# yifita/pytorch_points

Measured on AMD Instinct MI355X. Metric: chamfer_fwd_bwd_point_pairs_per_s, higher is better.
Workload: dtype f32

## Files before the change

### pytorch_points_amd/csrc/grid_common.h

```cpp
#pragma once
#include "pp_common.h"

#ifndef PP_PHASE
#define PP_PHASE(n)
#endif

namespace pp {

constexpr int kGridMax = 32;
constexpr float kGridMinExtent = 0x1p-44f;
constexpr int kGridCells = kGridMax * kGridMax * kGridMax;
constexpr int kBuildThreads = 1024;

constexpr int kBuildSlabs = 4;

constexpr int kLayerWords = 40;
constexpr int kLayerPending = 36;
constexpr int kLayerCursor = 37;
constexpr int kLayerRouted = 38;
constexpr int kChunk = 256;
constexpr int kChunkMax = 256;
__host__ __device__ inline int zkey(float z) {
#if defined(__HIP_DEVICE_COMPILE__)
  const int o = __float_as_int(z);
#else
  int o;
  __builtin_memcpy(&o, &z, 4);
#endif
  return o ^ ((o >> 31) & 0x7fffffff);
}
__device__ __forceinline__ float zkey_inv(int k) { return __int_as_float(k ^ ((k >> 31) & 0x7fffffff)); }

struct GridSet {
  float minx, miny, minz, h, invh;
  int gx, gy, gz;
  int useless;
  int pad[3];
  int crowd[kBuildSlabs];
};
static_assert(sizeof(GridSet) == 64, "");

__device__ __forceinline__ bool grid_useless(const GridSet& g) {
  return g.useless != 0 || g.crowd[0] == 1 || g.crowd[1] == 1 || g.crowd[2] == 1 || g.crowd[3] == 1;
}
__device__ __forceinline__ bool grid_refined(const GridSet& g) {
  return g.crowd[0] == 2 || g.crowd[1] == 2 || g.crowd[2] == 2 || g.crowd[3] == 2;
}

constexpr int kCrowd = 128;
constexpr int kSubMaxAxis = 26;
constexpr int kSubMaxCells = 16384;
constexpr int kSubWaveCells = 1536;
constexpr int kBuildSlabCrowdMax = 1024;
struct SubGrid {
  float minx, miny, minz, h, invh;
  int gx, gy, gz;
};
static_assert(sizeof(SubGrid) == 32, "");
__host__ __device__ inline size_t sub_desc_slots(size_t npoints) { return npoints / kCrowd + 2; }

__device__ __forceinline__ int cell_coord(float p, float mn, float invh, int g) {
  const float f = (p - mn) * invh;
  const int c = (int)f;
  int r;
  asm("v_med3_i32 %0, %1, 0, %2" : "=v"(r) : "v"(c), "v"(g - 1));
  return r;
}

__device__ __forceinline__ int cell_linear(int cx, int cy, int cz, int gx, int gy) {
  int r;
  asm("v_mad_u32_u24 %0, %1, %2, %3\n\tv_mad_u32_u24 %0, %0, %4, %5"
      : "=&v"(r)
      : "v"(cz), "v"(gy), "v"(cy), "v"(gx), "v"(cx));
  return r;
}

__host__ __device__ inline int grid_build_counter_words(int nslab) {
  const int per = (kGridCells + nslab - 1) / nslab + 1;
  return (per + per / 32 + 1 + 3) & ~3;
}
__host__ __device__ inline size_t grid_build_lds_bytes(int nslab) {
  return ((size_t)grid_build_counter_words(nslab) + (size_t)kBuildThreads * 16) * sizeof(unsigned);
}

__device__ __forceinline__ int morton3(int x, int y, int z) {
  auto spread = [](unsigned v) {
    v = (v | (v << 8)) & 0x0000f00fu;
    v = (v | (v << 4)) & 0x000c30c3u;
    v = (v | (v << 2)) & 0x00249249u;
    return v;
  };
  return (int)(spread((unsigned)x) | (spread((unsigned)y) << 1) | (spread((unsigned)z) << 2));
}

__device__ __attribute__((noinline)) void grid_refine_cells(f4* __restrict__ sorted, f4* __restrict__ sorted2,
                                                            float* __restrict__ sorted_payload,
                                                            float* __restrict__ payload2,
                                                            unsigned* __restrict__ sub_start,
                                                            SubGrid* __restrict__ sub_desc, unsigned* s_cnt,
                                                            unsigned* s_part, float* s_box,
                                                            const unsigned (*s_clist)[2], unsigned ncrowd) {
  const int t = threadIdx.x;
  {
    {
      const int lane = t & 63, wave = t >> 6;
      constexpr unsigned kWaveMaxPoints = 2048;
      auto sub_geometry = [&](const float (&bmn)[6], unsigned n, int max_cells) {
        SubGrid sg;
        sg.minx = -bmn[0]; sg.miny = -bmn[1]; sg.minz = -bmn[2];
        const float sex = bmn[3] - sg.minx, sey = bmn[4] - sg.miny, sez = bmn[5] - sg.minz;
        const float semax = fmaxf(sex, fmaxf(sey, sez));
        int g2 = (int)cbrtf((float)n);
        g2 = g2 < 2 ? 2 : (g2 > kSubMaxAxis - 1 ? kSubMaxAxis - 1 : g2);
        sg.h = semax / (float)g2;
        if (!(sg.h > 0.0f) || !__builtin_isfinite(sg.h) || semax < kGridMinExtent) sg.h = 1.0f;
        sg.invh = 1.0f / sg.h;
        auto cells2 = [&](float e) {
          const int c = (int)(e * sg.invh) + 1;
          return c < 1 ? 1 : (c > kSubMaxAxis ? kSubMaxAxis : c);
        };
        sg.gx = cells2(sex); sg.gy = cells2(sey); sg.gz = cells2(sez);
        while ((long long)sg.gx * sg.gy * sg.gz > min((long long)max_cells, 2LL * n - 1)) {
          if (sg.gx >= sg.gy && sg.gx >= sg.gz) --sg.gx; else if (sg.gy >= sg.gz) --sg.gy; else --sg.gz;
        }
        return sg;
      };
      auto trim_box = [&](float (&bmn)[6], const float (&sm)[6], unsigned n) {
        const float inv_n = 1.0f / (float)n;
        float lo[3] = {-bmn[0], -bmn[1], -bmn[2]}, hi[3] = {bmn[3], bmn[4], bmn[5]};
        const float ext0 = fmaxf(hi[0] - lo[0], fmaxf(hi[1] - lo[1], hi[2] - lo[2]));
        float tl[3], th[3];
#pragma unroll
        for (int a = 0; a < 3; ++a) {
          const float c = 0.5f * (lo[a] + hi[a]);
          const float m = sm[a] * inv_n;
          const float var = fmaxf(sm[3 + a] * inv_n - m * m, 0.0f);
          const float sd = sqrtf(var);
          tl[a] = fmaxf(lo[a], c + m - 3.5f * sd);
          th[a] = fminf(hi[a], c + m + 3.5f * sd);
        }
        const float ext1 = fmaxf(th[0] - tl[0], fmaxf(th[1] - tl[1], th[2] - tl[2]));
        if (ext1 > 0.0f && ext1 < 0.75f * ext0) {
#pragma unroll
          for (int a = 0; a < 3; ++a) {
            bmn[a] = -tl[a];
            bmn[3 + a] = th[a];
          }
        }
      };
      auto cell2 = [](const SubGrid& sg, const f4& p) {
        return cell_linear(cell_coord(p.x, sg.minx, sg.invh, sg.gx), cell_coord(p.y, sg.miny, sg.invh, sg.gy),
                           cell_coord(p.z, sg.minz, sg.invh, sg.gz), sg.gx, sg.gy);
      };
      auto wave_sync = []() {
        __builtin_amdgcn_fence(__ATOMIC_ACQ_REL, "workgroup");
        __builtin_amdgcn_wave_barrier();
      };
      {
        unsigned* s_sub = s_cnt + (size_t)wave * kSubWaveCells;
        for (unsigned ci = wave; ci < ncrowd; ci += kBuildThreads / 64) {
          const unsigned start = s_clist[ci][0], n = s_clist[ci][1];
          if (n > kWaveMaxPoints) continue;
          auto for_points = [&](const f4* __restrict__ src, auto&& fn) {
            for (unsigned k0 = 0; k0 < n; k0 += 512u) {
              f4 q8[8];
#pragma unroll
              for (int u = 0; u < 8; ++u) q8[u] = src[start + min(k0 + 64u * (unsigned)u + (unsigned)lane, n - 1u)];
#pragma unroll
              for (int u = 0; u < 8; ++u) {
                const unsigned k = k0 + 64u * (unsigned)u + (unsigned)lane;
                if (k < n) fn(q8[u], k);
              }
            }
          };
          float bmn[6] = {-__builtin_inff(), -__builtin_inff(), -__builtin_inff(), -__builtin_inff(), -__builtin_inff(),
                          -__builtin_inff()};
          for_points(sorted, [&](const f4& q, unsigned) {
            bmn[0] = fmaxf(bmn[0], -q.x); bmn[1] = fmaxf(bmn[1], -q.y); bmn[2] = fmaxf(bmn[2], -q.z);
            bmn[3] = fmaxf(bmn[3], q.x); bmn[4] = fmaxf(bmn[4], q.y); bmn[5] = fmaxf(bmn[5], q.z);
          });
          wave_reduce6_dpp<false, 6>(bmn);
#pragma unroll
          for (int e = 0; e < 6; ++e) bmn[e] = __int_as_float(__builtin_amdgcn_readlane(__float_as_int(bmn[e]), 63));
          {
            const float c0 = 0.5f * (bmn[3] - bmn[0]), c1 = 0.5f * (bmn[4] - bmn[1]), c2 = 0.5f * (bmn[5] - bmn[2]);
            float sm[6] = {0.0f, 0.0f, 0.0f, 0.0f, 0.0f, 0.0f};
            for_points(sorted, [&](const f4& q, unsigned) {
              const float dx = q.x - c0, dy = q.y - c1, dz = q.z - c2;
              sm[0] += dx; sm[1] += dy; sm[2] += dz;
              sm[3] = __builtin_fmaf(dx, dx, sm[3]); sm[4] = __builtin_fmaf(dy, dy, sm[4]); sm[5] = __builtin_fmaf(dz, dz, sm[5]);
            });
            wave_reduce6_dpp<true, 6>(sm);
#pragma unroll
            for (int e = 0; e < 6; ++e) sm[e] = __int_as_float(__builtin_amdgcn_readlane(__float_as_int(sm[e]), 63));
            trim_box(bmn, sm, n);
          }
          const SubGrid sg = sub_geometry(bmn, n, kSubWaveCells);
          const int total2 = sg.gx * sg.gy * sg.gz;
          for (int c = lane; c < total2; c += 64) s_sub[c] = 0u;
          wave_sync();
          for_points(sorted, [&](const f4& q, unsigned) { atomicAdd(&s_sub[cell2(sg, q)], 1u); });
          wave_sync();
          {
            const int per2 = (total2 + 63) / 64;
            const int d0 = min(total2, lane * per2), d1 = min(total2, d0 + per2);
            unsigned sum2 = 0;
            for (int c = d0; c < d1; ++c) sum2 += s_sub[c];
            unsigned incl2 = sum2;
#pragma unroll
            for (int off = 1; off < 64; off <<= 1) {
              const unsigned o = __shfl_up(incl2, off);
              if (lane >= off) incl2 += o;
            }
            unsigned run2 = start + incl2 - sum2;
            unsigned* __restrict__ tbl = sub_start + 2 * (size_t)start;
            for (int c = d0; c < d1; ++c) {
              const unsigned v = s_sub[c];
              s_sub[c] = run2;
              tbl[c] = run2;
              run2 += v;
            }
            if (lane == 0) tbl[total2] = start + n;
          }
          wave_sync();
          for_points(sorted, [&](const f4& q, unsigned k) {
            const unsigned pos = atomicAdd(&s_sub[cell2(sg, q)], 1u);
// ... 696 lines not shown
constexpr int kFastLdsCnt = 0;
constexpr int kFastLdsList = kFastLdsCnt + kFastCells + 64;
constexpr int kFastLdsTz = kFastLdsList + (kFastCap + 64) * 4;
constexpr int kFastLdsBox = kFastLdsTz + 2 * kChunkMax;
constexpr int kFastLdsPart = kFastLdsBox + (kBuildThreads / 64) * 16;
constexpr int kFastLdsClist = kFastLdsPart + 64;
constexpr int kFastLdsPlan = kFastLdsClist + 2 * kFastCrowdMax;
constexpr int kFastLdsWords = kFastLdsPlan + 16;
static_assert(sizeof(BuildPlan) <= 16 * 4, "");
__host__ __device__ inline size_t grid_build_fast_lds_bytes() { return (size_t)kFastLdsWords * 4; }

template <bool REFINE = true>
__device__ __forceinline__ int grid_build_set_fast(const float* __restrict__ ref, int nr, GridSet* gs,
                                                   unsigned* __restrict__ cell_start, f4* __restrict__ sorted,
                                                   unsigned* lds, int slab, unsigned* __restrict__ sub_start,
                                                   SubGrid* __restrict__ sub_desc, f4* __restrict__ sorted2,
                                                   int* __restrict__ tile_z, int tz_chunks,
                                                   unsigned* __restrict__ layers) {
  constexpr int KP = 16, nslab = kBuildSlabs;
  const int nchunkq = (nr + kChunk - 1) / kChunk;
  if (nr > kFastMaxPoints || nr < 4 * kBuildThreads || (nr & 3) != 0 || cell_start == nullptr) return 1;
  if (REFINE && (tile_z == nullptr || layers == nullptr || sub_start == nullptr || sub_desc == nullptr ||
                 nchunkq > tz_chunks || tz_chunks > kChunkMax))
    return 1;
  const int t = threadIdx.x, lane = t & 63, wave = __builtin_amdgcn_readfirstlane(t >> 6);
  unsigned* s_cnt = lds + kFastLdsCnt;
  f4* s_list = reinterpret_cast<f4*>(lds + kFastLdsList);
  unsigned* s_occ = lds + kFastLdsList;
  int* s_tz = reinterpret_cast<int*>(lds + kFastLdsTz);
  float* s_box = reinterpret_cast<float*>(lds + kFastLdsBox);
  unsigned* s_part = lds + kFastLdsPart;
  unsigned(*s_clist)[2] = reinterpret_cast<unsigned(*)[2]>(lds + kFastLdsClist);
  unsigned& s_below = s_part[33];
  unsigned& s_ncrowd = s_part[34];

  PP_PHASE(0);
  float px[KP], py[KP], pz[KP];
  bool live[KP / 4];
#pragma unroll
  for (int gq = 0; gq < KP / 4; ++gq) {
    const int p0 = gq * (4 * kBuildThreads) + 4 * t;
    live[gq] = p0 < nr;
    const f4* __restrict__ src = reinterpret_cast<const f4*>(ref + 3 * (size_t)(live[gq] ? p0 : 0));
    const f4 a = src[0], b = src[1], c = src[2];
    px[4 * gq] = a.x; py[4 * gq] = a.y; pz[4 * gq] = a.z;
    px[4 * gq + 1] = a.w; py[4 * gq + 1] = b.x; pz[4 * gq + 1] = b.y;
    px[4 * gq + 2] = b.z; py[4 * gq + 2] = b.w; pz[4 * gq + 2] = c.x;
    px[4 * gq + 3] = c.y; py[4 * gq + 3] = c.z; pz[4 * gq + 3] = c.w;
  }
  auto kidx = [&](int i) { return (i >> 2) * (4 * kBuildThreads) + 4 * t + (i & 3); };
  if (REFINE && t < 2 * kChunkMax) s_tz[t] = (t & 1) ? zkey(-__builtin_inff()) : zkey(__builtin_inff());
  if (t == 0) {
    s_ncrowd = 0u;
    s_below = 0u;
  }
  s_occ[t] = 0u;
  for (int c = 4 * t; c < kFastCells; c += 4 * kBuildThreads) *reinterpret_cast<uint4*>(&s_cnt[c]) = make_uint4(0u, 0u, 0u, 0u);
  float mnx = __builtin_inff(), mny = mnx, mnz = mnx, mxx = -mnx, mxy = -mnx, mxz = -mnx;
  float sm[6] = {0.0f, 0.0f, 0.0f, 0.0f, 0.0f, 0.0f};
#pragma unroll
  for (int i = 0; i < KP; ++i) {
    const float x = px[i], y = py[i], z = pz[i];
    mnx = fminf(mnx, x); mny = fminf(mny, y); mnz = fminf(mnz, z);
    mxx = fmaxf(mxx, x); mxy = fmaxf(mxy, y); mxz = fmaxf(mxz, z);
    if (live[i >> 2]) {
      sm[0] += x; sm[1] += y; sm[2] += z;
      sm[3] = __builtin_fmaf(x, x, sm[3]); sm[4] = __builtin_fmaf(y, y, sm[4]); sm[5] = __builtin_fmaf(z, z, sm[5]);
    }
  }
  PP_PHASE(1);
  bool any_bad;
  {
    float v[6] = {-mnx, -mny, -mnz, mxx, mxy, mxz};
    wave_reduce6_dpp<false, 6>(v);
    wave_reduce6_dpp<true, 6>(sm);
    if (lane == 63) {
#pragma unroll
      for (int e = 0; e < 6; ++e) s_box[wave * 16 + e] = v[e];
#pragma unroll
      for (int e = 0; e < 6; ++e) s_box[wave * 16 + 8 + e] = sm[e];
    }
    __syncthreads();
#pragma unroll
    for (int e = 0; e < 6; ++e) v[e] = s_box[(t & 15) * 16 + e];
#pragma unroll
    for (int e = 0; e < 6; ++e) sm[e] = s_box[(t & 15) * 16 + 8 + e];
    wave_reduce6_dpp<false, 4>(v);
    wave_reduce6_dpp<true, 4>(sm);
#pragma unroll
    for (int e = 0; e < 6; ++e) v[e] = __int_as_float(__builtin_amdgcn_readlane(__float_as_int(v[e]), 15));
#pragma unroll
    for (int e = 0; e < 6; ++e) sm[e] = __int_as_float(__builtin_amdgcn_readlane(__float_as_int(sm[e]), 15));
    mnx = -v[0]; mny = -v[1]; mnz = -v[2]; mxx = v[3]; mxy = v[4]; mxz = v[5];
    any_bad = !__builtin_isfinite(sm[3] + sm[4] + sm[5]);
  }
  float n_live = (float)nr;
  if (!REFINE && any_bad) {
    plain_finite_plan(ref, nr, s_box);
    auto uni = [&](int e) { return __int_as_float(__builtin_amdgcn_readfirstlane(__float_as_int(s_box[e]))); };
    mnx = -uni(0); mny = -uni(1); mnz = -uni(2); mxx = uni(3); mxy = uni(4); mxz = uni(5);
#pragma unroll
    for (int e = 0; e < 6; ++e) sm[e] = uni(8 + e);
    n_live = uni(14);
    any_bad = !(n_live > 0.0f) || !__builtin_isfinite(sm[3] + sm[4] + sm[5]);
    __syncthreads();
  }
  PP_PHASE(2);
  bool trimmed = false;
  float zmean = 0.0f, zsig = 0.0f;
  if (!any_bad) {
    const float inv_n = 1.0f / n_live;
    const float mean[3] = {sm[0] * inv_n, sm[1] * inv_n, sm[2] * inv_n};
    float sig[3];
#pragma unroll
    for (int a = 0; a < 3; ++a) sig[a] = sqrtf(fmaxf(sm[3 + a] * inv_n - mean[a] * mean[a], 0.0f));
    zmean = mean[2];
    zsig = sig[2];
    const bool stretched = mxx - mean[0] > 6.0f * sig[0] || mean[0] - mnx > 6.0f * sig[0] ||
                           mxy - mean[1] > 6.0f * sig[1] || mean[1] - mny > 6.0f * sig[1] ||
                           mxz - mean[2] > 6.0f * sig[2] || mean[2] - mnz > 6.0f * sig[2];
    if (stretched) {
      float w[6] = {-__builtin_inff(), -__builtin_inff(), -__builtin_inff(), -__builtin_inff(), -__builtin_inff(),
                    -__builtin_inff()};
#pragma unroll
      for (int i = 0; i < KP; ++i) {
        const float x = px[i], y = py[i], z = pz[i];
        const bool in = fabsf(x - mean[0]) <= 4.0f * sig[0] && fabsf(y - mean[1]) <= 4.0f * sig[1] &&
                        fabsf(z - mean[2]) <= 4.0f * sig[2];
        if (in) {
          w[0] = fmaxf(w[0], -x); w[1] = fmaxf(w[1], -y); w[2] = fmaxf(w[2], -z);
          w[3] = fmaxf(w[3], x); w[4] = fmaxf(w[4], y); w[5] = fmaxf(w[5], z);
        }
      }
#pragma unroll
      for (int e = 0; e < 6; ++e) w[e] = wave_reduce_dpp<false>(w[e]);
      __syncthreads();
      if (lane == 0)
#pragma unroll
        for (int e = 0; e < 6; ++e) s_box[wave * 16 + e] = w[e];
      __syncthreads();
#pragma unroll
      for (int e = 0; e < 6; ++e) w[e] = wave_reduce_dpp<false>(s_box[(t & 15) * 16 + e]);
      if (w[3] > -w[0] || w[4] > -w[1] || w[5] > -w[2]) {
        mnx = -w[0]; mny = -w[1]; mnz = -w[2]; mxx = w[3]; mxy = w[4]; mxz = w[5];
        trimmed = true;
      }
    }
  }
  PP_PHASE(3);
  const float ex = mxx - mnx, ey = mxy - mny, ez = mxz - mnz;
  const float emax = fmaxf(ex, fmaxf(ey, ez));
  if (any_bad || !(emax > 0.0f) || !__builtin_isfinite(emax) || emax < kGridMinExtent) return 1;
  int g0 = 1;
  while (g0 < kGridMax && g0 * g0 * g0 < 2 * nr) ++g0;
  float h, invh;
  int gx, gy, gz;
  auto set_resolution = [&](int g) {
    h = emax / (float)g;
    if (!(h > 0.0f) || !__builtin_isfinite(h)) h = 1.0f;
    invh = 1.0f / h;
    auto cells = [&](float e) {
      int c = (int)(e * invh) + 1;
      return c < 1 ? 1 : (c > kGridMax ? kGridMax : c);
    };
    gx = cells(ex); gy = cells(ey); gz = cells(ez);
  };
  set_resolution(g0);
  unsigned key[KP];
  int gxy = 0, lo = 0, ncs = 0;
  auto count_pass = [&](bool mark) {
    float ox = mnx, oy = mny, oz = mnz;
    asm volatile("" : "+s"(ox), "+s"(oy), "+s"(oz));
    unsigned nbelow = 0;
#pragma unroll
    for (int gq = 0; gq < KP / 4; ++gq) {
      int c4[4];
#pragma unroll
      for (int u = 0; u < 4; ++u) {
        const int i = 4 * gq + u;
        c4[u] = cell_linear(cell_coord(px[i], ox, invh, gx), cell_coord(py[i], oy, invh, gy),
                            cell_coord(pz[i], oz, invh, gz), gx, gy);
      }
      const bool alive = live[gq];
      const bool same4 = alive & (c4[0] == c4[1]) & (c4[1] == c4[2]) & (c4[2] == c4[3]);
      const int lead = __builtin_amdgcn_readfirstlane(c4[0]);
      if (__all(same4 && c4[0] == lead)) {
        const unsigned slot = (unsigned)(lead - lo);
        if (mark && lane == 0) atomicOr(&s_occ[lead >> 5], 1u << (lead & 31));
        if (lead < lo) nbelow += 256u;
        unsigned b0 = 0u;
        const bool mine = slot < (unsigned)ncs;
        if (mine && lane == 0) b0 = atomicAdd(&s_cnt[slot], 256u);
        b0 = (unsigned)__builtin_amdgcn_readfirstlane((int)b0) + 4u * (unsigned)lane;
#pragma unroll
        for (int u = 0; u < 4; ++u) key[4 * gq + u] = mine ? (slot | ((b0 + (unsigned)u) << 16)) : ~0u;
      } else {
#pragma unroll
        for (int u = 0; u < 4; ++u) {
          const int c = c4[u];
          if (mark) atomicOr(&s_occ[c >> 5], 1u << (c & 31));
          const unsigned slot = (unsigned)(c - lo);
          const bool mine = alive & (slot < (unsigned)ncs);
          nbelow += (unsigned)__builtin_popcountll(__ballot(alive & (c < lo)));
          const unsigned r = atomicAdd(&s_cnt[mine ? slot : (unsigned)(kFastCells + lane)], 1u);
          key[4 * gq + u] = mine ? (slot | (r << 16)) : ~0u;
        }
      }
    }
    if (lane == 0 && nbelow) atomicAdd(&s_below, nbelow);
  };
  unsigned running = 0, own = 0;
#if PP_BUILD_BALANCE
  const bool balance_z = fabsf(zsig - 0.2887f * ez) > 0.03f * ez || fabsf(zmean - (mnz + 0.5f * ez)) > 0.06f * ez;
#endif
  {
    constexpr int kRounds = 4;
    for (int round = 0;; ++round) {
      if (gz < kFastMinLayers) return 1;
      gxy = gx * gy;
      int zl = gz * slab / nslab, zh = gz * (slab + 1) / nslab;
#if PP_BUILD_BALANCE
      if (balance_z) {
        unsigned* s_hist = reinterpret_cast<unsigned*>(s_box);
        if (t < 32) s_hist[t] = 0u;
        __syncthreads();
#pragma unroll
        for (int gq = 0; gq < KP / 4; ++gq)
          if (live[gq]) atomicAdd(&s_hist[cell_coord(pz[4 * gq], mnz, invh, gz)], 1u);
        __syncthreads();
        const unsigned cum = wave_scan_u32_dpp(lane < gz ? s_hist[lane] : 0u);
        const unsigned tot = (unsigned)__builtin_amdgcn_readlane((int)cum, 63);
        int zb[nslab + 1];
        zb[0] = 0;
        zb[nslab] = gz;
#pragma unroll
        for (int k = 1; k < nslab; ++k)
          zb[k] = min(max((int)__builtin_popcountll(__ballot(lane < gz && (unsigned)nslab * cum <= (unsigned)k * tot)), zb[k - 1] + 1),
                      gz - (nslab - k));
        bool fits = true;
#pragma unroll
        for (int k = 0; k < nslab; ++k) fits = fits && (zb[k + 1] - zb[k]) * gxy <= kFastCells;
        if (fits) {
#pragma unroll
          for (int k = 0; k < nslab; ++k)
            if (k == slab) {
              zl = zb[k];
              zh = zb[k + 1];
            }
        }
      }
#endif
      lo = zl * gxy;
      ncs = (zh - zl) * gxy;
      const int nwords = (gxy * gz + 31) / 32;
      if (round > 0) {
        if (t < nwords) s_occ[t] = 0u;
        for (int c = 4 * t; c < ((ncs + 7) & ~7); c += 4 * kBuildThreads)
          *reinterpret_cast<uint4*>(&s_cnt[c]) = make_uint4(0u, 0u, 0u, 0u);
        if (t == 0) s_below = 0u;
        __syncthreads();
      }
      PP_PHASE(4);
      count_pass(round < kRounds);
      __syncthreads();
      PP_PHASE(5);
      unsigned v8[8];
      const int c0 = 8 * t;
      if (c0 < ncs) {
        const uint4 a = *reinterpret_cast<const uint4*>(&s_cnt[c0]);
        const uint4 b = *reinterpret_cast<const uint4*>(&s_cnt[c0 + 4]);
        v8[0] = a.x; v8[1] = a.y; v8[2] = a.z; v8[3] = a.w; v8[4] = b.x; v8[5] = b.y; v8[6] = b.z; v8[7] = b.w;
      } else {
#pragma unroll
        for (int u = 0; u < 8; ++u) v8[u] = 0u;
      }
      unsigned sum = 0;
#pragma unroll
      for (int u = 0; u < 8; ++u) sum += v8[u];
      const unsigned incl = wave_scan_u32_dpp(sum);
      const unsigned occ = wave_scan_u32_dpp(round < kRounds && t < nwords ? (unsigned)__builtin_popcount(s_occ[t]) : 0u);
      if (lane == 63) {
        s_part[wave] = incl;
        s_part[16 + wave] = occ;
      }
      __syncthreads();
      const unsigned tot16 = wave_scan_u32_dpp(s_part[lane & 15]);
      const unsigned occ16 = wave_scan_u32_dpp(s_part[16 + (lane & 15)]);
      const unsigned nocc = (unsigned)__builtin_amdgcn_readlane((int)occ16, 15);
      const int gmax = max(gx, max(gy, gz));
      if (round < kRounds && !((float)nr >= 2.5f * (float)nocc || gmax <= 4)) {
        int gn = max(4, (int)((float)gmax * 0.7071f));
#if PP_BUILD_JUMP
        {
          const float lam = 2.0f * ((float)nr / (float)nocc - 1.0f);
          const float want = (float)gmax * (float)gmax * (float)gmax * lam * (1.0f / 2.6f);
          while (gn > 4 && (float)gn * (float)gn * (float)gn > want) --gn;
        }
#endif
        set_resolution(gn);
        __syncthreads();
        continue;
      }
      const unsigned wbase = wave == 0 ? 0u : (unsigned)__builtin_amdgcn_readlane((int)tot16, (wave - 1) & 15);
      own = (unsigned)__builtin_amdgcn_readlane((int)tot16, 15);
      running = s_below;
      if (t == 0) {
        BuildPlan* plan = reinterpret_cast<BuildPlan*>(lds + kFastLdsPlan);
        plan->mnx = mnx; plan->mny = mny; plan->mnz = mnz; plan->h = h; plan->invh = invh;
        plan->gx = gx; plan->gy = gy; plan->gz = gz; plan->cell_lo = lo; plan->cell_hi = lo + ncs; plan->trimmed = trimmed ? 1 : 0;
      }
#if !PP_BUILD_SPILL
      if (own > (unsigned)kFastCap) return 2;
#endif
      unsigned run = running + wbase + incl - sum;
      if (c0 < ncs) {
        unsigned st[8], mx8 = 0u;
#pragma unroll
        for (int u = 0; u < 8; ++u) {
          st[u] = run;
          run += v8[u];
          mx8 = max(mx8, v8[u]);
        }
        if (!REFINE) {
          if ((float)mx8 > 256.0f + (float)nr * (1.0f / 32.0f)) atomicOr(&s_ncrowd, 1u);
        } else if (mx8 > (unsigned)kCrowd) {
#pragma unroll
          for (int u = 0; u < 8; ++u)
            if (v8[u] > (unsigned)kCrowd) {
              const unsigned at = atomicAdd(&s_ncrowd, 1u);
              if (at < (unsigned)kFastCrowdMax) {
                s_clist[at][0] = st[u];
                s_clist[at][1] = v8[u];
              }
            }
        }
        *reinterpret_cast<uint4*>(&s_cnt[c0]) = make_uint4(st[0], st[1], st[2], st[3]);
        *reinterpret_cast<uint4*>(&s_cnt[c0 + 4]) = make_uint4(st[4], st[5], st[6], st[7]);
      }
      break;
    }
  }
  const int ncell = gxy * gz;
  const int zl = lo / gxy, zh = (lo + ncs) / gxy;
  __syncthreads();
  PP_PHASE(6);
  if (((lo | ncs) & 3) == 0 && (reinterpret_cast<uintptr_t>(cell_start) & 15) == 0) {
    for (int c = 4 * t; c < ncs; c += 4 * kBuildThreads)
      *reinterpret_cast<uint4*>(&cell_start[lo + c]) = *reinterpret_cast<const uint4*>(&s_cnt[c]);
  } else {
    for (int c = t; c < ncs; c += kBuildThreads) cell_start[lo + c] = s_cnt[c];
  }
  if (REFINE && t < zh - zl) layers[zl + t] = s_cnt[t * gxy];
  const bool spill = PP_BUILD_SPILL && own > (unsigned)kFastCap;
#pragma unroll
  for (int i = 0; i < KP; ++i) {
    const bool mine = key[i] != ~0u;
#if PP_BUILD_STAGE_MASKED
    if (mine) {
      const unsigned pos = s_cnt[key[i] & 0xffffu] + (key[i] >> 16) - running;
      f4 r = {px[i], py[i], pz[i], __int_as_float(kidx(i))};
      if (spill) {
        sorted[pos + running] = r;
        if (REFINE) {
          const unsigned ch = (pos + running) / (unsigned)kChunk;
          atomicMin(&s_tz[2 * ch], zkey(pz[i]));
          atomicMax(&s_tz[2 * ch + 1], zkey(pz[i]));
        }
      } else {
        s_list[pos] = r;
      }
    }
#else
    const unsigned start = s_cnt[mine ? (key[i] & 0xffffu) : 0u];
    const unsigned pos = mine ? start + (key[i] >> 16) - running : (unsigned)(kFastCap + lane);
    f4 r = {px[i], py[i], pz[i], __int_as_float(kidx(i))};
    s_list[pos] = r;
#endif
  }
  __syncthreads();
  PP_PHASE(7);
  if (own > 0u && !spill) {
    const unsigned ch_first = running / (unsigned)kChunk, ch_last = (running + own - 1u) / (unsigned)kChunk;
    for (unsigned ch = ch_first + (unsigned)wave; ch <= ch_last; ch += (unsigned)(kBuildThreads / 64)) {
      float zmax = -__builtin_inff(), nzmin = -__builtin_inff();
      const unsigned p0 = ch * (unsigned)kChunk;
      if (p0 >= running && p0 + (unsigned)kChunk <= running + own) {
#pragma unroll
        for (int q = 0; q < kChunk / 64; ++q) {
          const unsigned pos = p0 + (unsigned)(q * 64 + lane);
          const f4 r = s_list[pos - running];
          sorted[pos] = r;
          zmax = fmaxf(zmax, r.z);
          nzmin = fmaxf(nzmin, -r.z);
        }
      } else {
#pragma unroll
        for (int q = 0; q < kChunk / 64; ++q) {
          const unsigned pos = p0 + (unsigned)(q * 64 + lane);
          const unsigned j = pos - running;
          const bool have = j < own;
          const f4 r = s_list[have ? j : 0u];
          if (have) {
            sorted[pos] = r;
            zmax = fmaxf(zmax, r.z);
            nzmin = fmaxf(nzmin, -r.z);
          }
        }
      }
      if (!REFINE) continue;
      zmax = wave_reduce_dpp<false>(zmax);
      nzmin = wave_reduce_dpp<false>(nzmin);
      if (lane == 0) {
        s_tz[2 * ch] = zkey(-nzmin);
        s_tz[2 * ch + 1] = zkey(zmax);
      }
    }
  }
  __syncthreads();
  PP_PHASE(8);
  PP_PHASE(9);
  const unsigned ncrowd = s_ncrowd;
  if (REFINE && ncrowd > (unsigned)kFastCrowdMax) return 2;
  if (t == 0 && slab == nslab - 1) {
    cell_start[ncell] = (unsigned)nr;
    if (REFINE) layers[gz] = (unsigned)nr;
  }
  bool refined = false;
  if constexpr (REFINE) {
    if ((t == kLayerPending || t == kLayerCursor || t == kLayerRouted) && slab == 0) layers[t] = 0u;
    for (int c = t; c < 2 * tz_chunks; c += kBuildThreads) tile_z[((size_t)(c >> 1) * nslab + slab) * 2 + (c & 1)] = s_tz[c];
    if (ncrowd > 0) {
      __threadfence_block();
      __syncthreads();
      refined = true;
      grid_refine_cells(sorted, sorted2, nullptr, nullptr, sub_start, sub_desc, reinterpret_cast<unsigned*>(s_list), s_cnt,
                        s_box, s_clist, ncrowd);
    }
  }
  if (t == 0) {
    gs->crowd[slab] = REFINE ? (refined ? 2 : 0) : (ncrowd != 0u ? 1 : 0);
    if (slab == 0) {
      gs->minx = mnx; gs->miny = mny; gs->minz = mnz; gs->h = h; gs->invh = invh;
      gs->gx = gx; gs->gy = gy; gs->gz = gz;
      gs->useless = 0;
      gs->pad[0] = 0;
      gs->pad[1] = REFINE ? 1 : 0;
      gs->pad[2] = trimmed ? 1 : 0;
    }
  }
  PP_PHASE(10);
  return 0;
}

template <bool MORTON, bool VEC>
__device__ __forceinline__ void grid_build_set(const float* __restrict__ ref, int nr, GridSet* gs,
                                               unsigned* __restrict__ cell_start, f4* __restrict__ sorted,
                                               int* __restrict__ inv, unsigned* s_cnt,
                                               const float* __restrict__ payload = nullptr,
                                               float* __restrict__ sorted_payload = nullptr, int slab = 0,
                                               int nslab = 1) {
  grid_build_set_impl<MORTON, VEC, false>(ref, nr, gs, cell_start, sorted, inv, s_cnt, payload, sorted_payload, slab,
                                          nslab, nullptr, nullptr, nullptr, nullptr);
}

template <bool VEC>
__device__ __forceinline__ void grid_build_set_plain(const float* __restrict__ ref, int nr, GridSet* gs,
                                                     unsigned* __restrict__ cell_start, f4* __restrict__ sorted,
                                                     unsigned* s_cnt, int slab, int nslab) {
  int how = 1;
#ifndef PP_PLAIN_GENERAL
  if constexpr (VEC) {
    if (nslab == kBuildSlabs)
      how = grid_build_set_fast<false>(ref, nr, gs, cell_start, sorted, s_cnt, slab, nullptr, nullptr, nullptr, nullptr, 0,
                                       nullptr);
  }
#endif
  if (how == 0) return;
  __syncthreads();
  grid_build_set_impl<false, VEC, false>(ref, nr, gs, cell_start, sorted, nullptr, s_cnt, nullptr, nullptr, slab, nslab, nullptr,
                                         nullptr, nullptr, nullptr, nullptr, 0, nullptr,
                                         how == 2 ? reinterpret_cast<const BuildPlan*>(s_cnt + kFastLdsPlan) : nullptr);
}

template <bool VEC>
__device__ __forceinline__ void grid_build_set_refined(const float* __restrict__ ref, int nr, GridSet* gs,
                                                       unsigned* __restrict__ cell_start, f4* __restrict__ sorted,
                                                       unsigned* s_cnt, const float* __restrict__ payload,
                                                       float* __restrict__ sorted_payload, int slab, int nslab,
                                                       unsigned* __restrict__ sub_start,
                                                       SubGrid* __restrict__ sub_desc, f4* __restrict__ sorted2,
                                                       float* __restrict__ payload2, int* __restrict__ tile_z = nullptr,
                                                       int tz_chunks = 0, unsigned* __restrict__ layers = nullptr) {
  grid_build_set_impl<false, VEC, true>(ref, nr, gs, cell_start, sorted, nullptr, s_cnt, payload, sorted_payload, slab,
                                        nslab, sub_start, sub_desc, sorted2, payload2, tile_z, tz_chunks, layers);
}

inline bool clouds_vec_aligned(const void* a, int na, int batch) {
  return (reinterpret_cast<uintptr_t>(a) & 15) == 0 && (batch <= 1 || na % 4 == 0);
}

}
```

### pytorch_points_amd/csrc/pp_common.h

```cpp
#pragma once
#include <hip/hip_runtime.h>
#include <stdint.h>

#include <atomic>
#include <type_traits>

#include "pp_hip.h"
#include "pp_hip_debug.h"

#define PP_WAVE 64

#define PP_RETURN_IF_LAUNCH_FAILED()        \
  do {                                      \
    hipError_t e__ = hipGetLastError();     \
    if (e__ != hipSuccess) return (int)e__; \
  } while (0)

namespace pp {

struct Knob {
  std::atomic<int> v{0};
  operator int() const { return v.load(std::memory_order_relaxed); }
  void set(int x) { v.store(x, std::memory_order_relaxed); }
};
struct DeviceFlags {
  std::atomic<bool> f[64] = {};
};

template <typename K>
inline hipError_t allow_big_lds(K kernel, int bytes, DeviceFlags& flags) {
  int dev = 0;
  hipError_t e = hipGetDevice(&dev);
  if (e != hipSuccess) {
    (void)hipGetLastError();
    return e;
  }
  if (dev < 0 || dev >= 64) dev = 63;
  if (dev != 63 && flags.f[dev].load(std::memory_order_acquire)) return hipSuccess;
  e = hipFuncSetAttribute((const void*)kernel, hipFuncAttributeMaxDynamicSharedMemorySize, bytes);
  if (e == hipSuccess)
    flags.f[dev].store(true, std::memory_order_release);
  else
    (void)hipGetLastError();
  return e;
}

template <int>
__global__ void fill_u32_kernel(unsigned* p, unsigned v, long long n) {
  for (long long i = (long long)blockIdx.x * blockDim.x + threadIdx.x; i < n; i += (long long)gridDim.x * blockDim.x) p[i] = v;
}
template <int>
__global__ void fill_u8_kernel(unsigned char* p, unsigned char v, long long n) {
  for (long long i = (long long)blockIdx.x * blockDim.x + threadIdx.x; i < n; i += (long long)gridDim.x * blockDim.x) p[i] = v;
}
inline hipError_t fill_bytes(void* p, unsigned char byte, size_t bytes, hipStream_t s) {
  if (bytes == 0) return hipSuccess;
  const bool words = ((uintptr_t)p & 3u) == 0 && (bytes & 3u) == 0;
  const long long n = words ? (long long)(bytes / 4) : (long long)bytes;
  const long long blocks = (n + 255) / 256 < 8192 ? (n + 255) / 256 : 8192;
  if (words)
    fill_u32_kernel<0><<<dim3((unsigned)blocks), dim3(256), 0, s>>>((unsigned*)p, 0x01010101u * byte, n);
  else
    fill_u8_kernel<0><<<dim3((unsigned)blocks), dim3(256), 0, s>>>((unsigned char*)p, byte, n);
  return hipGetLastError();
}

__device__ __forceinline__ float chamfer_d3(float rx, float ry, float rz, float qx, float qy,
                                            float qz) {
  const float t0 = rx - qx, t1 = ry - qy, t2 = rz - qz;
  return __builtin_fmaf(t2, t2, __builtin_fmaf(t1, t1, t0 * t0));
}

typedef float f2 __attribute__((ext_vector_type(2)));
typedef float f4 __attribute__((ext_vector_type(4)));
typedef int i4 __attribute__((ext_vector_type(4)));

__device__ __forceinline__ f2 chamfer_d3_pk(float rx, float ry, float rz, f2 qx, f2 qy, f2 qz) {
  const f2 t0 = (f2)(rx) - qx, t1 = (f2)(ry) - qy, t2 = (f2)(rz) - qz;
  return __builtin_elementwise_fma(t2, t2, __builtin_elementwise_fma(t1, t1, t0 * t0));
}

__device__ __forceinline__ float dist3(float ax, float ay, float az, float bx, float by, float bz) {
  const float dx = ax - bx, dy = ay - by, dz = az - bz;
  return __builtin_fmaf(dz, dz, __builtin_fmaf(dx, dx, dy * dy));
}

__device__ __forceinline__ f2 dist3_pk(float ax, float ay, float az, f2 bx, f2 by, f2 bz) {
  const f2 dx = (f2)(ax) - bx, dy = (f2)(ay) - by, dz = (f2)(az) - bz;
  return __builtin_elementwise_fma(dz, dz, __builtin_elementwise_fma(dx, dx, dy * dy));
}

template <typename KEY, typename SWAP>
__device__ __forceinline__ void lane_sort(unsigned n, KEY key, SWAP swap) {
  if (n < 2) return;
  if (n <= 24) {
    for (unsigned i = 1; i < n; ++i)
      for (unsigned j = i; j > 0 && key(j - 1) > key(j); --j) swap(j - 1, j);
    return;
  }
  auto sift = [&](unsigned root, unsigned end) {
    for (;;) {
      unsigned child = 2 * root + 1;
      if (child >= end) return;
      if (child + 1 < end && key(child + 1) > key(child)) ++child;
      if (!(key(child) > key(root))) return;
      swap(root, child);
      root = child;
    }
  };
  for (unsigned i = n / 2; i-- > 0;) sift(i, n);
  for (unsigned end = n - 1; end > 0; --end) {
    swap(0, end);
    sift(0, end);
  }
}

__device__ __forceinline__ float min3(float a, float b, float c) {
  float r;
  asm("v_min3_f32 %0, %1, %2, %3" : "=v"(r) : "v"(a), "v"(b), "v"(c));
  return r;
}

template <bool SUM>
__device__ __forceinline__ float wave_reduce_dpp(float v) {
  auto step = [](float x, auto ctrl, auto row_mask) {
    const float o = __int_as_float(__builtin_amdgcn_update_dpp(SUM ? 0 : __float_as_int(x), __float_as_int(x),
                                                               decltype(ctrl)::value, decltype(row_mask)::value,
                                                               0xf, false));
    return SUM ? x + o : fmaxf(x, o);
  };
  using I = std::integral_constant<int, 0>;
  (void)sizeof(I);
  v = step(v, std::integral_constant<int, 0x111>{}, std::integral_constant<int, 0xf>{});
  v = step(v, std::integral_constant<int, 0x112>{}, std::integral_constant<int, 0xf>{});
  v = step(v, std::integral_constant<int, 0x114>{}, std::integral_constant<int, 0xf>{});
  v = step(v, std::integral_constant<int, 0x118>{}, std::integral_constant<int, 0xf>{});
  v = step(v, std::integral_constant<int, 0x142>{}, std::integral_constant<int, 0xa>{});
  v = step(v, std::integral_constant<int, 0x143>{}, std::integral_constant<int, 0xc>{});
  return __int_as_float(__builtin_amdgcn_readlane(__float_as_int(v), 63));
}

#define PP_DPP6_STEP(OP, CTRL)                                                                       \
  OP " %0, %0, %0 " CTRL "\n\t" OP " %1, %1, %1 " CTRL "\n\t" OP " %2, %2, %2 " CTRL "\n\t" OP     \
     " %3, %3, %3 " CTRL "\n\t" OP " %4, %4, %4 " CTRL "\n\t" OP " %5, %5, %5 " CTRL "\n\t"
#define PP_DPP6_ROWS(OP)                                                                             \
  "s_nop 1\n\t" PP_DPP6_STEP(OP, "row_shr:1 row_mask:0xf bank_mask:0xf")                            \
      PP_DPP6_STEP(OP, "row_shr:2 row_mask:0xf bank_mask:0xf")                                       \
          PP_DPP6_STEP(OP, "row_shr:4 row_mask:0xf bank_mask:0xf")                                   \
              PP_DPP6_STEP(OP, "row_shr:8 row_mask:0xf bank_mask:0xf")
#define PP_DPP6_WAVE(OP)                                                                             \
  PP_DPP6_ROWS(OP) PP_DPP6_STEP(OP, "row_bcast:15 row_mask:0xa bank_mask:0xf")                       \
      PP_DPP6_STEP(OP, "row_bcast:31 row_mask:0xc bank_mask:0xf")
template <bool SUM, int STEPS>
__device__ __forceinline__ void wave_reduce6_dpp(float (&v)[6]) {
  static_assert(STEPS == 4 || STEPS == 6, "");
  if constexpr (SUM && STEPS == 6)
    asm volatile(PP_DPP6_WAVE("v_add_f32_dpp") "s_nop 1" : "+v"(v[0]), "+v"(v[1]), "+v"(v[2]), "+v"(v[3]), "+v"(v[4]), "+v"(v[5]));
  else if constexpr (SUM)
    asm volatile(PP_DPP6_ROWS("v_add_f32_dpp") "s_nop 1" : "+v"(v[0]), "+v"(v[1]), "+v"(v[2]), "+v"(v[3]), "+v"(v[4]), "+v"(v[5]));
  else if constexpr (STEPS == 6)
    asm volatile(PP_DPP6_WAVE("v_max_f32_dpp") "s_nop 1" : "+v"(v[0]), "+v"(v[1]), "+v"(v[2]), "+v"(v[3]), "+v"(v[4]), "+v"(v[5]));
  else
    asm volatile(PP_DPP6_ROWS("v_max_f32_dpp") "s_nop 1" : "+v"(v[0]), "+v"(v[1]), "+v"(v[2]), "+v"(v[3]), "+v"(v[4]), "+v"(v[5]));
}

#define PP_DPP1_WAVE(OP)                                                                             \
  "s_nop 1\n\t" OP " %0, %0, %0 row_shr:1 row_mask:0xf bank_mask:0xf\n\t"                          \
  "s_nop 1\n\t" OP " %0, %0, %0 row_shr:2 row_mask:0xf bank_mask:0xf\n\t"                          \
  "s_nop 1\n\t" OP " %0, %0, %0 row_shr:4 row_mask:0xf bank_mask:0xf\n\t"                          \
  "s_nop 1\n\t" OP " %0, %0, %0 row_shr:8 row_mask:0xf bank_mask:0xf\n\t"                          \
  "s_nop 1\n\t" OP " %0, %0, %0 row_bcast:15 row_mask:0xa bank_mask:0xf\n\t"                       \
  "s_nop 1\n\t" OP " %0, %0, %0 row_bcast:31 row_mask:0xc bank_mask:0xf\n\t"                       \
  "s_nop 1"
__device__ __forceinline__ unsigned wave_max_u32_dpp1(unsigned v) {
  asm volatile(PP_DPP1_WAVE("v_max_u32_dpp") : "+v"(v));
  return (unsigned)__builtin_amdgcn_readlane((int)v, 63);
}
__device__ __forceinline__ unsigned wave_min_u32_dpp1(unsigned v) {
  asm volatile(PP_DPP1_WAVE("v_min_u32_dpp") : "+v"(v));
  return (unsigned)__builtin_amdgcn_readlane((int)v, 63);
}
__device__ __forceinline__ unsigned long long wave_min_u64_dpp1(unsigned long long key) {
  const unsigned hi = (unsigned)(key >> 32), lo = (unsigned)key;
  const unsigned mh = wave_min_u32_dpp1(hi);
  const unsigned ml = wave_min_u32_dpp1(hi == mh ? lo : 0xffffffffu);
  return ((unsigned long long)mh << 32) | ml;
}

__device__ __forceinline__ unsigned wave_min_u32_dpp(unsigned v) {
#define PP_MIN_STEP(CTRL, ROWS)                                                                  \
  {                                                                                               \
    const unsigned o = (unsigned)__builtin_amdgcn_update_dpp((int)v, (int)v, CTRL, ROWS, 0xf, false); \
    v = o < v ? o : v;                                                                            \
  }
  PP_MIN_STEP(0x111, 0xf)
  PP_MIN_STEP(0x112, 0xf)
  PP_MIN_STEP(0x114, 0xf)
  PP_MIN_STEP(0x118, 0xf)
  PP_MIN_STEP(0x142, 0xa)
  PP_MIN_STEP(0x143, 0xc)
#undef PP_MIN_STEP
  return (unsigned)__builtin_amdgcn_readlane((int)v, 63);
}
__device__ __forceinline__ unsigned long long wave_min_u64_dpp(unsigned long long key) {
  const unsigned hi = (unsigned)(key >> 32), lo = (unsigned)key;
  const unsigned mh = wave_min_u32_dpp(hi);
  const unsigned ml = wave_min_u32_dpp(hi == mh ? lo : 0xffffffffu);
  return ((unsigned long long)mh << 32) | ml;
}

__device__ __forceinline__ int wave_id_uniform() {
  return __builtin_amdgcn_readfirstlane((int)(threadIdx.x >> 6));
}

__device__ __forceinline__ int xcd_virtual_block(int linear, int per_xcd) {
  return (linear & 7) * per_xcd + (linear >> 3);
}

}
```

Measured before the change: 250100 billion.

## Micro-optimize grid build count and scatter passes with scalar operands and batched atomics

Several small changes to the grid-build kernel. The grid-resolution search becomes a binary search. Cell-coordinate math takes scalar-register operands. The uniform-cell check uses ballots compared to exec. Per-point LDS atomics are batched without the dummy-slot atomic. The running offset is folded in at write-out rather than into every prefix entry, the scatter is split by spill path, and two wave reductions are fused into one interleaved DPP sequence. Together these aim to trim instruction count and LDS traffic in the build phase. The risk is subtle correctness bugs in offset handling, since 'running' now moves into other places.

```diff
diff --git a/pytorch_points_amd/csrc/grid_common.h b/pytorch_points_amd/csrc/grid_common.h
--- a/pytorch_points_amd/csrc/grid_common.h
+++ b/pytorch_points_amd/csrc/grid_common.h
@@ -72,6 +72,21 @@
   asm("v_mad_u32_u24 %0, %1, %2, %3\n\tv_mad_u32_u24 %0, %0, %4, %5"
       : "=&v"(r)
       : "v"(cz), "v"(gy), "v"(cy), "v"(gx), "v"(cx));
+  return r;
+}
+
+__device__ __forceinline__ int cell_coord_s(float p, float mn, float invh, int gm1) {
+  const float f = (p - mn) * invh;
+  const int c = (int)f;
+  int r;
+  asm("v_med3_i32 %0, %1, 0, %2" : "=v"(r) : "v"(c), "s"(gm1));
+  return r;
+}
+__device__ __forceinline__ int cell_linear_s(int cx, int cy, int cz, int gx, int gy) {
+  int r;
+  asm("v_mad_u32_u24 %0, %1, %2, %3\n\tv_mad_u32_u24 %0, %0, %4, %5"
+      : "=&v"(r)
+      : "v"(cz), "s"(gy), "v"(cy), "s"(gx), "v"(cx));
   return r;
 }
 
@@ -1074,7 +1089,15 @@
   const float emax = fmaxf(ex, fmaxf(ey, ez));
   if (any_bad || !(emax > 0.0f) || !__builtin_isfinite(emax) || emax < kGridMinExtent) return 1;
   int g0 = 1;
-  while (g0 < kGridMax && g0 * g0 * g0 < 2 * nr) ++g0;
+  {
+    int ghi = kGridMax;
+#pragma unroll
+    for (int s = 0; s < 5; ++s) {
+      const int mid = (g0 + ghi) >> 1;
+      if (mid * mid * mid >= 2 * nr) ghi = mid; else g0 = mid + 1;
+    }
+  }
+  static_assert(kGridMax == 32, "five halvings");
   float h, invh;
   int gx, gy, gz;
   auto set_resolution = [&](int g) {
@@ -1088,11 +1111,16 @@
     gx = cells(ex); gy = cells(ey); gz = cells(ez);
   };
   set_resolution(g0);
+  constexpr unsigned kForeign = 0xffff0000u;
+  static_assert(kFastMaxPoints < 0xffff && kFastCells <= 0x10000, "rank and slot share a word");
   unsigned key[KP];
   int gxy = 0, lo = 0, ncs = 0;
-  auto count_pass = [&](bool mark) {
+  auto count_pass = [&]() {
     float ox = mnx, oy = mny, oz = mnz;
     asm volatile("" : "+s"(ox), "+s"(oy), "+s"(oz));
+    const int gxm1 = __builtin_amdgcn_readfirstlane(gx - 1), gym1 = __builtin_amdgcn_readfirstlane(gy - 1),
+              gzm1 = __builtin_amdgcn_readfirstlane(gz - 1);
+    const int sgx = __builtin_amdgcn_readfirstlane(gx), sgy = __builtin_amdgcn_readfirstlane(gy);
     unsigned nbelow = 0;
 #pragma unroll
     for (int gq = 0; gq < KP / 4; ++gq) {
@@ -1100,32 +1128,42 @@
 #pragma unroll
       for (int u = 0; u < 4; ++u) {
         const int i = 4 * gq + u;
-        c4[u] = cell_linear(cell_coord(px[i], ox, invh, gx), cell_coord(py[i], oy, invh, gy),
-                            cell_coord(pz[i], oz, invh, gz), gx, gy);
+        c4[u] = cell_linear_s(cell_coord_s(px[i], ox, invh, gxm1), cell_coord_s(py[i], oy, invh, gym1),
+                              cell_coord_s(pz[i], oz, invh, gzm1), sgx, sgy);
       }
       const bool alive = live[gq];
-      const bool same4 = alive & (c4[0] == c4[1]) & (c4[1] == c4[2]) & (c4[2] == c4[3]);
       const int lead = __builtin_amdgcn_readfirstlane(c4[0]);
-      if (__all(same4 && c4[0] == lead)) {
+      const unsigned long long same4 = __builtin_amdgcn_ballot_w64(alive) & __builtin_amdgcn_ballot_w64(c4[0] == c4[1]) &
+                                       __builtin_amdgcn_ballot_w64(c4[1] == c4[2]) & __builtin_amdgcn_ballot_w64(c4[2] == c4[3]) &
+                                       __builtin_amdgcn_ballot_w64(c4[0] == lead);
+      if (same4 == __builtin_amdgcn_read_exec()) {
         const unsigned slot = (unsigned)(lead - lo);
-        if (mark && lane == 0) atomicOr(&s_occ[lead >> 5], 1u << (lead & 31));
+        if (lane == 0) atomicOr(&s_occ[lead >> 5], 1u << (lead & 31));
         if (lead < lo) nbelow += 256u;
         unsigned b0 = 0u;
         const bool mine = slot < (unsigned)ncs;
         if (mine && lane == 0) b0 = atomicAdd(&s_cnt[slot], 256u);
         b0 = (unsigned)__builtin_amdgcn_readfirstlane((int)b0) + 4u * (unsigned)lane;
 #pragma unroll
-        for (int u = 0; u < 4; ++u) key[4 * gq + u] = mine ? (slot | ((b0 + (unsigned)u) << 16)) : ~0u;
+        for (int u = 0; u < 4; ++u) key[4 * gq + u] = mine ? (slot | ((b0 + (unsigned)u) << 16)) : kForeign;
       } else {
+        unsigned r4[4];
 #pragma unroll
         for (int u = 0; u < 4; ++u) {
+          asm volatile("" : "=v"(r4[u]));
           const int c = c4[u];
-          if (mark) atomicOr(&s_occ[c >> 5], 1u << (c & 31));
+          atomicOr(&s_occ[c >> 5], 1u << (c & 31));
           const unsigned slot = (unsigned)(c - lo);
           const bool mine = alive & (slot < (unsigned)ncs);
           nbelow += (unsigned)__builtin_popcountll(__ballot(alive & (c < lo)));
-          const unsigned r = atomicAdd(&s_cnt[mine ? slot : (unsigned)(kFastCells + lane)], 1u);
-          key[4 * gq + u] = mine ? (slot | (r << 16)) : ~0u;
+          if (mine) r4[u] = atomicAdd(&s_cnt[slot], 1u);
+        }
+#pragma unroll
+        for (int u = 0; u < 4; ++u) {
+          asm volatile("" : "+v"(r4[u]));
+          const unsigned slot = (unsigned)(c4[u] - lo);
+          const bool mine = alive & (slot < (unsigned)ncs);
+          key[4 * gq + u] = mine ? (slot | (r4[u] << 16)) : kForeign;
         }
       }
     }
@@ -1183,7 +1221,7 @@
         __syncthreads();
       }
       PP_PHASE(4);
-      count_pass(round < kRounds);
+      count_pass();
       __syncthreads();
       PP_PHASE(5);
       unsigned v8[8];
@@ -1234,7 +1272,7 @@
 #if !PP_BUILD_SPILL
       if (own > (unsigned)kFastCap) return 2;
 #endif
-      unsigned run = running + wbase + incl - sum;
+      unsigned run = wbase + incl - sum;
       if (c0 < ncs) {
         unsigned st[8], mx8 = 0u;
 #pragma unroll
@@ -1251,7 +1289,7 @@
             if (v8[u] > (unsigned)kCrowd) {
               const unsigned at = atomicAdd(&s_ncrowd, 1u);
               if (at < (unsigned)kFastCrowdMax) {
-                s_clist[at][0] = st[u];
+                s_clist[at][0] = running + st[u];
                 s_clist[at][1] = v8[u];
               }
             }
@@ -1267,38 +1305,50 @@
   __syncthreads();
   PP_PHASE(6);
   if (((lo | ncs) & 3) == 0 && (reinterpret_cast<uintptr_t>(cell_start) & 15) == 0) {
+    typedef unsigned u4 __attribute__((ext_vector_type(4)));
     for (int c = 4 * t; c < ncs; c += 4 * kBuildThreads)
-      *reinterpret_cast<uint4*>(&cell_start[lo + c]) = *reinterpret_cast<const uint4*>(&s_cnt[c]);
+      *reinterpret_cast<u4*>(&cell_start[lo + c]) = *reinterpret_cast<const u4*>(&s_cnt[c]) + running;
   } else {
-    for (int c = t; c < ncs; c += kBuildThreads) cell_start[lo + c] = s_cnt[c];
-  }
-  if (REFINE && t < zh - zl) layers[zl + t] = s_cnt[t * gxy];
+    for (int c = t; c < ncs; c += kBuildThreads) cell_start[lo + c] = running + s_cnt[c];
+  }
+  if (REFINE && t < zh - zl) layers[zl + t] = running + s_cnt[t * gxy];
   const bool spill = PP_BUILD_SPILL && own > (unsigned)kFastCap;
-#pragma unroll
-  for (int i = 0; i < KP; ++i) {
-    const bool mine = key[i] != ~0u;
 #if PP_BUILD_STAGE_MASKED
-    if (mine) {
-      const unsigned pos = s_cnt[key[i] & 0xffffu] + (key[i] >> 16) - running;
-      f4 r = {px[i], py[i], pz[i], __int_as_float(kidx(i))};
-      if (spill) {
-        sorted[pos + running] = r;
+  if (!spill) {
+#pragma unroll
+    for (int gq = 0; gq < KP / 4; ++gq) {
+      unsigned start[4];
+#pragma unroll
+      for (int u = 0; u < 4; ++u) start[u] = s_cnt[key[4 * gq + u] & 0xffffu];
+#pragma unroll
+      for (int u = 0; u < 4; ++u) {
+        const int i = 4 * gq + u;
+        unsigned pos = start[u] + (key[i] >> 16);
+        asm("" : "+v"(pos));
+        if (key[i] < kForeign) s_list[pos] = f4{px[i], py[i], pz[i], __int_as_float(kidx(i))};
+      }
+    }
+  } else {
+#pragma unroll
+    for (int i = 0; i < KP; ++i)
+      if (key[i] < kForeign) {
+        const unsigned pos = running + s_cnt[key[i] & 0xffffu] + (key[i] >> 16);
+        sorted[pos] = f4{px[i], py[i], pz[i], __int_as_float(kidx(i))};
         if (REFINE) {
-          const unsigned ch = (pos + running) / (unsigned)kChunk;
+          const unsigned ch = pos / (unsigned)kChunk;
           atomicMin(&s_tz[2 * ch], zkey(pz[i]));
           atomicMax(&s_tz[2 * ch + 1], zkey(pz[i]));
         }
-      } else {
-        s_list[pos] = r;
-      }
-    }
+      }
+  }
 #else
-    const unsigned start = s_cnt[mine ? (key[i] & 0xffffu) : 0u];
-    const unsigned pos = mine ? start + (key[i] >> 16) - running : (unsigned)(kFastCap + lane);
-    f4 r = {px[i], py[i], pz[i], __int_as_float(kidx(i))};
-    s_list[pos] = r;
+#pragma unroll
+  for (int i = 0; i < KP; ++i) {
+    const bool mine = key[i] < kForeign;
+    const unsigned pos = mine ? s_cnt[key[i] & 0xffffu] + (key[i] >> 16) : (unsigned)(kFastCap + lane);
+    s_list[pos] = f4{px[i], py[i], pz[i], __int_as_float(kidx(i))};
+  }
 #endif
-  }
   __syncthreads();
   PP_PHASE(7);
   if (own > 0u && !spill) {
@@ -1330,8 +1380,7 @@
         }
       }
       if (!REFINE) continue;
-      zmax = wave_reduce_dpp<false>(zmax);
-      nzmin = wave_reduce_dpp<false>(nzmin);
+      wave_max2_dpp(zmax, nzmin);
       if (lane == 0) {
         s_tz[2 * ch] = zkey(-nzmin);
         s_tz[2 * ch + 1] = zkey(zmax);
diff --git a/pytorch_points_amd/csrc/pp_common.h b/pytorch_points_amd/csrc/pp_common.h
--- a/pytorch_points_amd/csrc/pp_common.h
+++ b/pytorch_points_amd/csrc/pp_common.h
@@ -164,6 +164,18 @@
     asm volatile(PP_DPP6_ROWS("v_max_f32_dpp") "s_nop 1" : "+v"(v[0]), "+v"(v[1]), "+v"(v[2]), "+v"(v[3]), "+v"(v[4]), "+v"(v[5]));
 }
 
+#define PP_DPP2_STEP(CTRL) \
+  "v_max_f32_dpp %0, %0, %0 " CTRL "\n\tv_max_f32_dpp %1, %1, %1 " CTRL "\n\ts_nop 0\n\t"
+__device__ __forceinline__ void wave_max2_dpp(float& a, float& b) {
+  asm volatile("s_nop 1\n\t" PP_DPP2_STEP("row_shr:1 row_mask:0xf bank_mask:0xf")
+                   PP_DPP2_STEP("row_shr:2 row_mask:0xf bank_mask:0xf") PP_DPP2_STEP("row_shr:4 row_mask:0xf bank_mask:0xf")
+                       PP_DPP2_STEP("row_shr:8 row_mask:0xf bank_mask:0xf") PP_DPP2_STEP("row_bcast:15 row_mask:0xa bank_mask:0xf")
+                           PP_DPP2_STEP("row_bcast:31 row_mask:0xc bank_mask:0xf") "s_nop 0"
+               : "+v"(a), "+v"(b));
+  a = __int_as_float(__builtin_amdgcn_readlane(__float_as_int(a), 63));
+  b = __int_as_float(__builtin_amdgcn_readlane(__float_as_int(b), 63));
+}
+
 #define PP_DPP1_WAVE(OP)                                                                             \
   "s_nop 1\n\t" OP " %0, %0, %0 row_shr:1 row_mask:0xf bank_mask:0xf\n\t"                          \
   "s_nop 1\n\t" OP " %0, %0, %0 row_shr:2 row_mask:0xf bank_mask:0xf\n\t"                          \
```

Result: no change. 252500 billion (median of 6 runs) (+1.0%).
